# rg2/DeepFluoroLabeling-IPCAI2020

Hardware: AMD Instinct MI355X
Metric: train images/sec, paper U-Net (depth 6, wf 5, BN, strided-conv down, seg + 14-landmark heads), 1x192x192 (8x-downsampled 184x184 padded) (higher is better)
Workload: dtype bf16 (bf16 activations, activation gradients and GEMM weight copies in HBM; bf16 MFMA, fp32 accumulate, BatchNorm statistics, losses, weight gradients and master weights); 1 GPU; BASELINE configs[1]: 8x-downsampled, seg + 14-landmark heat-map dual head, batch 16 per GPU, Dice+NCC loss, SGD nesterov; global_batch=16, image=1x192x192, parallelism=dp1, math=bf16s, optimizer=dfl_amd.SGD(momentum 0.9, nesterov, wd 1e-4)

## Files before the change

### deepfluorolabeling-ipcai2020_amd/csrc/direct_small.hip

```cpp
#include "common.h"
#include "direct_small.h"

namespace dfl {

constexpr int DK = DIRECT_MAX_K;

struct Gather {
  int iy0, ix0, base;
};

struct PixCursor {
  int ox, oy, n;
  __device__ __forceinline__ void init(int m, int Hg, int Wg) {
    ox = m % Wg;
    const int t = m / Wg;
    oy = t % Hg;
    n = t / Hg;
  }
  __device__ __forceinline__ void advance(int step, int Hg, int Wg) {
    ox += step;
    while (ox >= Wg) {
      ox -= Wg;
      if (++oy == Hg) {
        oy = 0;
        ++n;
      }
    }
  }
  __device__ __forceinline__ Gather origin(int stride, int pad, int Hin, int Win) const {
    Gather g;
    g.iy0 = oy * stride - pad;
    g.ix0 = ox * stride - pad;
    g.base = n * Hin * Win;
    return g;
  }
};

template <bool BF>
__device__ __forceinline__ float4 ld4c(const float* base, int64_t elem) {
  if constexpr (BF) {
    const uint2 w = *reinterpret_cast<const uint2*>(reinterpret_cast<const unsigned short*>(base) + elem);
    return make_float4(__uint_as_float(w.x << 16), __uint_as_float(w.x & 0xffff0000u), __uint_as_float(w.y << 16),
                       __uint_as_float(w.y & 0xffff0000u));
  } else {
    return *reinterpret_cast<const float4*>(base + elem);
  }
}
template <bool BF>
__device__ __forceinline__ float4 st4c(float* base, int64_t elem, float4 v) {
  if constexpr (BF) {
    const bf16x2_t h0 = __builtin_convertvector((f32x2_t){v.x, v.y}, bf16x2_t), h1 = __builtin_convertvector((f32x2_t){v.z, v.w}, bf16x2_t);
    const uint2 w = make_uint2(__builtin_bit_cast(unsigned, h0), __builtin_bit_cast(unsigned, h1));
    *reinterpret_cast<uint2*>(reinterpret_cast<unsigned short*>(base) + elem) = w;
    return make_float4(__uint_as_float(w.x << 16), __uint_as_float(w.x & 0xffff0000u), __uint_as_float(w.y << 16),
                       __uint_as_float(w.y & 0xffff0000u));
  } else {
    *reinterpret_cast<float4*>(base + elem) = v;
    return v;
  }
}

template <int KH, int KW, int CIN, bool BF>
__global__ void __launch_bounds__(256) direct_conv_kernel(const dfl_conv_args a, int Mtot, int rows_per_block) {
  constexpr int K = KH * KW * CIN;
  static_assert(K <= DK, "window too large for the direct kernel");
  __shared__ float red[2][256][4];
  const int cq = a.Ntot / 4, PL = 256 / cq;
  const int q = threadIdx.x % cq, pl = threadIdx.x / cq;
  const int n0 = 4 * q;
  float w[K][4];
#pragma unroll
  for (int k = 0; k < K; ++k) {
#pragma unroll
    for (int j = 0; j < 4; ++j) w[k][j] = a.w[((int64_t)(k >> 2) * a.Ntot + n0 + j) * 4 + (k & 3)];
  }
  float bias[4] = {0.f, 0.f, 0.f, 0.f}, asc[4] = {1.f, 1.f, 1.f, 1.f}, ash[4] = {0.f, 0.f, 0.f, 0.f};
#pragma unroll
  for (int j = 0; j < 4; ++j) {
    if (a.bias != nullptr) bias[j] = a.bias[n0 + j];
    if (a.add_scale != nullptr) {
      asc[j] = a.add_scale[n0 + j];
      ash[j] = a.add_shift[n0 + j];
    }
  }
  if (a.add != nullptr && a.add_scale == nullptr && a.add_tot != nullptr) {
    __shared__ float atab[2][1024];
    for (int c = threadIdx.x; c < a.Ntot; c += 256)
      bn_live_affine(a.add_tot, a.add_gamma, a.add_beta, a.add_count, a.bn_eps, a.Ntot, c, &atab[0][c], &atab[1][c]);
    __syncthreads();
#pragma unroll
    for (int j = 0; j < 4; ++j) {
      asc[j] = atab[0][n0 + j];
      ash[j] = atab[1][n0 + j];
    }
  }
  float isc[CIN], ish[CIN];
#pragma unroll
  for (int c = 0; c < CIN; ++c) {
    isc[c] = (a.in_scale != nullptr) ? a.in_scale[c] : 1.f;
    ish[c] = (a.in_scale != nullptr) ? a.in_shift[c] : 0.f;
  }
  float s1[4] = {0.f, 0.f, 0.f, 0.f}, s2[4] = {0.f, 0.f, 0.f, 0.f};
  const int m_begin = blockIdx.x * rows_per_block;
  const int m_end = min(Mtot, m_begin + rows_per_block);
  PixCursor cur;
  cur.init(min(m_begin + pl, Mtot - 1), a.Hout, a.Wout);
  for (int m = m_begin + pl; m < m_end; m += PL, cur.advance(PL, a.Hout, a.Wout)) {
    const Gather g = cur.origin(a.stride, a.pad, a.Hin, a.Win);
    float acc[4] = {bias[0], bias[1], bias[2], bias[3]};
    float xv[K];
#pragma unroll
    for (int dy = 0; dy < KH; ++dy)
#pragma unroll
      for (int dx = 0; dx < KW; ++dx)
#pragma unroll
        for (int c = 0; c < CIN; ++c) {
          const int iy = g.iy0 + dy, ix = g.ix0 + dx;
          const bool ok = (unsigned)iy < (unsigned)a.Hin && (unsigned)ix < (unsigned)a.Win;
          const float x = a.x[ok ? ((int64_t)(g.base + iy * a.Win + ix) * a.ldx + c) : 0];
          xv[(dy * KW + dx) * CIN + c] = ok ? fmaf(x, isc[c], ish[c]) : 0.f;
        }
#pragma unroll
    for (int k = 0; k < K; ++k)
#pragma unroll
      for (int j = 0; j < 4; ++j) acc[j] = fmaf(xv[k], w[k][j], acc[j]);
    if (a.add != nullptr) {
      const float4 r = ld4c<BF>(a.add, (int64_t)m * a.ldadd + n0);
      acc[0] += fmaf(r.x, asc[0], ash[0]);
      acc[1] += fmaf(r.y, asc[1], ash[1]);
      acc[2] += fmaf(r.z, asc[2], ash[2]);
      acc[3] += fmaf(r.w, asc[3], ash[3]);
    }
    if (a.relu) {
#pragma unroll
      for (int j = 0; j < 4; ++j) acc[j] = fmaxf(acc[j], 0.f);
    }
    const int64_t yo = (int64_t)m * a.ldy + n0;
    if (a.accumulate) {
      const float4 o = ld4c<BF>(a.y, yo);
      acc[0] += o.x; acc[1] += o.y; acc[2] += o.z; acc[3] += o.w;
    }
    const float4 st = st4c<BF>(a.y, yo, make_float4(acc[0], acc[1], acc[2], acc[3]));
    acc[0] = st.x; acc[1] = st.y; acc[2] = st.z; acc[3] = st.w;
    if (a.stat_partials != nullptr) {
      float u[4] = {acc[0], acc[1], acc[2], acc[3]};
      if (a.stat_other != nullptr) {
        const float4 o = ld4c<BF>(a.stat_other, (int64_t)m * a.ldso + n0);
        u[0] = o.x; u[1] = o.y; u[2] = o.z; u[3] = o.w;
      }
#pragma unroll
      for (int j = 0; j < 4; ++j) {
        s1[j] += acc[j];
        s2[j] = fmaf(acc[j], u[j], s2[j]);
      }
    }
  }
  if (a.stat_partials == nullptr) return;
#pragma unroll
  for (int j = 0; j < 4; ++j) {
    red[0][threadIdx.x][j] = s1[j];
    red[1][threadIdx.x][j] = s2[j];
  }
  __syncthreads();
  if (pl == 0) {
#pragma unroll
    for (int j = 0; j < 4; ++j) {
      float t1 = 0.f, t2 = 0.f;
      for (int p = 0; p < PL; ++p) {
        t1 += red[0][p * cq + q][j];
        t2 += red[1][p * cq + q][j];
      }
      a.stat_partials[((int64_t)blockIdx.x * 2 + 0) * a.Ntot + n0 + j] = t1;
      a.stat_partials[((int64_t)blockIdx.x * 2 + 1) * a.Ntot + n0 + j] = t2;
    }
  }
}

template <bool BF>
__device__ __forceinline__ void ld8c(const float* base, int64_t elem, float* v) {
  if constexpr (BF) {
    const uint4 w = *reinterpret_cast<const uint4*>(reinterpret_cast<const unsigned short*>(base) + elem);
    v[0] = __uint_as_float(w.x << 16); v[1] = __uint_as_float(w.x & 0xffff0000u);
    v[2] = __uint_as_float(w.y << 16); v[3] = __uint_as_float(w.y & 0xffff0000u);
    v[4] = __uint_as_float(w.z << 16); v[5] = __uint_as_float(w.z & 0xffff0000u);
    v[6] = __uint_as_float(w.w << 16); v[7] = __uint_as_float(w.w & 0xffff0000u);
  } else {
    const float4 a = *reinterpret_cast<const float4*>(base + elem), b = *reinterpret_cast<const float4*>(base + elem + 4);
    v[0] = a.x; v[1] = a.y; v[2] = a.z; v[3] = a.w; v[4] = b.x; v[5] = b.y; v[6] = b.z; v[7] = b.w;
  }
}
template <bool BF>
__device__ __forceinline__ void st8c(float* base, int64_t elem, float* v) {
  if constexpr (BF) {
    uint4 w;
    w.x = __builtin_bit_cast(unsigned, __builtin_convertvector((f32x2_t){v[0], v[1]}, bf16x2_t));
    w.y = __builtin_bit_cast(unsigned, __builtin_convertvector((f32x2_t){v[2], v[3]}, bf16x2_t));
    w.z = __builtin_bit_cast(unsigned, __builtin_convertvector((f32x2_t){v[4], v[5]}, bf16x2_t));
    w.w = __builtin_bit_cast(unsigned, __builtin_convertvector((f32x2_t){v[6], v[7]}, bf16x2_t));
    *reinterpret_cast<uint4*>(reinterpret_cast<unsigned short*>(base) + elem) = w;
    v[0] = __uint_as_float(w.x << 16); v[1] = __uint_as_float(w.x & 0xffff0000u);
    v[2] = __uint_as_float(w.y << 16); v[3] = __uint_as_float(w.y & 0xffff0000u);
    v[4] = __uint_as_float(w.z << 16); v[5] = __uint_as_float(w.z & 0xffff0000u);
    v[6] = __uint_as_float(w.w << 16); v[7] = __uint_as_float(w.w & 0xffff0000u);
  } else {
    *reinterpret_cast<float4*>(base + elem) = make_float4(v[0], v[1], v[2], v[3]);
    *reinterpret_cast<float4*>(base + elem + 4) = make_float4(v[4], v[5], v[6], v[7]);
  }
}

#ifndef DFL_ROWS_CONV_RB
#define DFL_ROWS_CONV_RB 2
#endif
#ifndef DFL_ROWS_WGRAD_RB
#define DFL_ROWS_WGRAD_RB 4
#endif
#ifndef DFL_ROWS_CONV_BPB
#define DFL_ROWS_CONV_BPB 3
#endif
#ifndef DFL_ROWS_WGRAD_BPB
#define DFL_ROWS_WGRAD_BPB 1
#endif
constexpr int ROWS_CONV_BPB = DFL_ROWS_CONV_BPB, ROWS_WGRAD_BPB = DFL_ROWS_WGRAD_BPB;
constexpr int ROWS_CONV_RB = DFL_ROWS_CONV_RB, ROWS_WGRAD_RB = DFL_ROWS_WGRAD_RB;

template <bool BF>
__global__ void __launch_bounds__(256) direct_conv3_rows_kernel(const dfl_conv_args a) {
  __shared__ float red[2][256][8];
  const int cq = a.Ntot >> 3, PL = 256 / cq;
  const int q = threadIdx.x % cq, pl = threadIdx.x / cq;
  const int n0 = 8 * q;
  const int bands = (a.Hout + ROWS_CONV_RB - 1) / ROWS_CONV_RB;
  float w[9][8], bias[8], s1[8], s2[8];
#pragma unroll
  for (int j = 0; j < 8; ++j) {
#pragma unroll
    for (int k = 0; k < 9; ++k) w[k][j] = a.w[((int64_t)(k >> 2) * a.Ntot + n0 + j) * 4 + (k & 3)];
    bias[j] = a.bias != nullptr ? a.bias[n0 + j] : 0.f;
    s1[j] = 0.f;
    s2[j] = 0.f;
  }
  extern __shared__ float img_rows[];
  const int RW = a.Wout + 2;
  for (int bb = 0; bb < ROWS_CONV_BPB; ++bb) {
  const int band = (int)blockIdx.x * ROWS_CONV_BPB + bb;
  if (band >= a.N * bands) break;
  const int n = band / bands, y0 = (band - n * bands) * ROWS_CONV_RB;
  const float* img = a.x + (int64_t)n * a.Hin * a.Win * a.ldx;
  if (bb > 0) __syncthreads();
  for (int idx = threadIdx.x; idx < (ROWS_CONV_RB + 2) * RW; idx += 256) {
    const int r = idx / RW, c = idx - r * RW;
    const int iy = y0 - a.pad + r, ix = c - a.pad;
    const bool ok = (unsigned)iy < (unsigned)a.Hin && (unsigned)ix < (unsigned)a.Win;
    img_rows[idx] = ok ? img[(int64_t)(iy * a.Win + ix) * a.ldx] : 0.f;
  }
  __syncthreads();
#pragma unroll
  for (int ry = 0; ry < ROWS_CONV_RB; ++ry) {
    const int y = y0 + ry;
    if (y >= a.Hout) break;
    for (int x = pl; x < a.Wout; x += PL) {
      float xv[9];
#pragma unroll
      for (int dy = 0; dy < 3; ++dy)
#pragma unroll
        for (int dx = 0; dx < 3; ++dx) xv[dy * 3 + dx] = img_rows[(ry + dy) * RW + x + dx];
      float acc[8];
#pragma unroll
      for (int j = 0; j < 8; ++j) acc[j] = bias[j];
#pragma unroll
      for (int k = 0; k < 9; ++k)
#pragma unroll
        for (int j = 0; j < 8; ++j) acc[j] = fmaf(xv[k], w[k][j], acc[j]);
      if (a.relu) {
#pragma unroll
        for (int j = 0; j < 8; ++j) acc[j] = fmaxf(acc[j], 0.f);
      }
      st8c<BF>(a.y, ((int64_t)(n * a.Hout + y) * a.Wout + x) * a.ldy + n0, acc);
#pragma unroll
      for (int j = 0; j < 8; ++j) {
        s1[j] += acc[j];
        s2[j] = fmaf(acc[j], acc[j], s2[j]);
      }
    }
  }
  if (a.stat_partials != nullptr || a.stat_totals != nullptr) {
    __syncthreads();
#pragma unroll
    for (int j = 0; j < 8; ++j) {
      red[0][threadIdx.x][j] = s1[j];
      red[1][threadIdx.x][j] = s2[j];
      s1[j] = 0.f;
      s2[j] = 0.f;
    }
    __syncthreads();
    for (int idx = threadIdx.x; idx < 2 * a.Ntot; idx += 256) {
      const int which = idx / a.Ntot, c = idx - which * a.Ntot;
      const int qq = c >> 3, j = c & 7;
      float t = 0.f;
      for (int p = 0; p < PL; ++p) t += red[which][p * cq + qq][j];
      if (a.stat_totals != nullptr) bn_live_add(a.stat_totals, band, which, a.Ntot, c, t);
      else a.stat_partials[((int64_t)band * 2 + which) * a.Ntot + c] = t;
    }
  }
  }
}

static bool direct_conv_rows_ok(const dfl_conv_args* a) {
  return a->KH == 3 && a->KW == 3 && a->Cin == 1 && a->stride == 1 && a->add == nullptr && !a->accumulate && a->stat_other == nullptr &&
         a->in_scale == nullptr && a->Ntot % 8 == 0 && a->Ntot <= 64 && 256 % (a->Ntot / 8) == 0 && a->ldy % 8 == 0 && aligned16(a->y);
}

template <bool BF, bool DB = false>
__global__ void __launch_bounds__(256) direct_wgrad3_rows_kernel(const dfl_wgrad_args a) {
  __shared__ float red[4][8 * 72];
  const int cq = a.Cm >> 3, PL = 256 / cq;
  const int q = threadIdx.x % cq, pl = threadIdx.x / cq;
  const int bands = (a.Hout + ROWS_WGRAD_RB - 1) / ROWS_WGRAD_RB;
  float acc[9][8];
#pragma unroll
  for (int k = 0; k < 9; ++k)
#pragma unroll
    for (int j = 0; j < 8; ++j) acc[k][j] = 0.f;
  extern __shared__ float img_rows[];
  const int RW = a.Wout + 2;
  float cA[DB ? 8 : 1], cB[DB ? 8 : 1], cC[DB ? 8 : 1], bsum[DB ? 8 : 1];
  if constexpr (DB) {
    if (a.coef_tot != nullptr) {
      float* ctab = &red[0][0];
      if ((int)threadIdx.x < a.Cm)
        bn_live_coef(a.coef_tot, a.bn_gamma, a.bn_mean, a.bn_invstd, a.bn_count, a.Cm, (int)threadIdx.x, ctab + threadIdx.x, ctab + 64 + threadIdx.x,
                     ctab + 128 + threadIdx.x);
      __syncthreads();
#pragma unroll
      for (int j = 0; j < 8; ++j) {
        cA[j] = ctab[8 * q + j];
        cB[j] = ctab[64 + 8 * q + j];
        cC[j] = ctab[128 + 8 * q + j];
        bsum[j] = 0.f;
      }
      __syncthreads();
    } else {
#pragma unroll
      for (int j = 0; j < 8; ++j) {
        cA[j] = a.coef != nullptr ? a.coef[8 * q + j] : 1.f;
        cB[j] = a.coef != nullptr ? a.coef[a.Cm + 8 * q + j] : 0.f;
        cC[j] = a.coef != nullptr ? a.coef[2 * a.Cm + 8 * q + j] : 0.f;
        bsum[j] = 0.f;
      }
    }
  }
  for (int bb = 0; bb < ROWS_WGRAD_BPB; ++bb) {
  const int band = (int)blockIdx.x * ROWS_WGRAD_BPB + bb;
  if (band >= a.N * bands) break;
  const int n = band / bands, y0 = (band - n * bands) * ROWS_WGRAD_RB;
  const float* img = a.g + (int64_t)n * a.Hin * a.Win * a.ldg;
  if (bb > 0) __syncthreads();
  for (int idx = threadIdx.x; idx < (ROWS_WGRAD_RB + 2) * RW; idx += 256) {
    const int r = idx / RW, c = idx - r * RW;
    const int iy = y0 - a.pad + r, ix = c - a.pad;
    const bool ok = (unsigned)iy < (unsigned)a.Hin && (unsigned)ix < (unsigned)a.Win;
    img_rows[idx] = ok ? img[(int64_t)(iy * a.Win + ix) * a.ldg] : 0.f;
  }
  __syncthreads();
#pragma unroll
  for (int ry = 0; ry < ROWS_WGRAD_RB; ++ry) {
    const int y = y0 + ry;
    if (y >= a.Hout) break;
    for (int x = pl; x < a.Wout; x += PL) {
      float d[8], xv[9];
      ld8c<BF>(a.d, ((int64_t)(n * a.Hout + y) * a.Wout + x) * a.ldd + 8 * q, d);
      if constexpr (DB) {
        float r[8];
        ld8c<BF>(a.d2, ((int64_t)(n * a.Hout + y) * a.Wout + x) * a.ldd2 + 8 * q, r);
#pragma unroll
        for (int j = 0; j < 8; ++j) {
          const float v = r[j] > 0.f ? fmaf(cA[j], d[j], fmaf(cB[j], r[j], cC[j])) : 0.f;
          d[j] = (float)(__bf16)v;
          bsum[j] += d[j];
        }
      }
#pragma unroll
      for (int dy = 0; dy < 3; ++dy)
#pragma unroll
        for (int dx = 0; dx < 3; ++dx) xv[dy * 3 + dx] = img_rows[(ry + dy) * RW + x + dx];
#pragma unroll
      for (int k = 0; k < 9; ++k)
#pragma unroll
        for (int j = 0; j < 8; ++j) acc[k][j] = fmaf(xv[k], d[j], acc[k][j]);
    }
  }
  }
  const int lane = threadIdx.x & 63, wave = threadIdx.x >> 6;
#pragma unroll
  for (int k = 0; k < 9; ++k)
#pragma unroll
    for (int j = 0; j < 8; ++j) {
      float v = acc[k][j];
      for (int off = cq; off < 64; off <<= 1) v += __shfl_xor(v, off, 64);
      acc[k][j] = v;
    }
  if (lane < cq) {
#pragma unroll
    for (int k = 0; k < 9; ++k)
#pragma unroll
      for (int j = 0; j < 8; ++j) red[wave][(lane * 9 + k) * 8 + j] = acc[k][j];
  }
  __syncthreads();
  const bool sliced = a.splits > 1;
  float* out = sliced ? a.partial + (int64_t)blockIdx.x * a.Cm * 9 : a.dw;
  for (int idx = threadIdx.x; idx < cq * 72; idx += 256) {
    const float t = ((red[0][idx] + red[1][idx]) + red[2][idx]) + red[3][idx];
    const int qq = idx / 72, r = idx - qq * 72, k = r >> 3, j = r & 7;
    const int cm = 8 * qq + j;
    out[sliced ? (int64_t)k * a.Cm + cm : (int64_t)cm * 9 + k] = t;
  }
  if constexpr (DB) {
    if (a.bias_partial == nullptr) return;
#pragma unroll
    for (int j = 0; j < 8; ++j) {
      float v = bsum[j];
      for (int off = cq; off < 64; off <<= 1) v += __shfl_xor(v, off, 64);
      bsum[j] = v;
    }
    __syncthreads();
    if (lane < cq) {
#pragma unroll
      for (int j = 0; j < 8; ++j) red[wave][lane * 8 + j] = bsum[j];
    }
    __syncthreads();
    for (int idx = threadIdx.x; idx < a.Cm; idx += 256)
      a.bias_partial[(int64_t)blockIdx.x * a.Cm + idx] = ((red[0][idx] + red[1][idx]) + red[2][idx]) + red[3][idx];
  }
}

static bool direct_wgrad_rows_ok(const dfl_wgrad_args* a) {
  return a->KH == 3 && a->KW == 3 && a->Cg == 1 && a->stride == 1 && a->in_scale == nullptr && a->Cm % 8 == 0 && a->Cm <= 64 &&
         256 % (a->Cm / 8) == 0 && 64 % (a->Cm / 8) == 0 && a->ldd % 8 == 0 && aligned16(a->d) && !a->g_bf16;
}

static bool direct_window(int KH, int KW, int C) {
  if (KH != KW) return false;
  return (KH == 3 && C == 1) || (KH == 2 && C >= 1 && C <= 3) || (KH == 1 && C >= 1 && C <= 4);
}

bool direct_conv_rows_usable(const dfl_conv_args* a) { return direct_conv_rows_ok(a); }

bool direct_conv_ok(const dfl_conv_args* a) {
  if (!direct_window(a->KH, a->KW, a->Cin) || a->scatter2x2 || a->splits > 1) return false;
  if (a->Ntot % 4 != 0 || a->Ntot > 1024 || 256 % (a->Ntot / 4) != 0) return false;
  if (a->x_bf16) return false;
  if (a->ldy % 4 != 0 || !aligned16(a->y)) return false;
  if (a->add != nullptr && (a->ldadd % 4 != 0 || !aligned16(a->add))) return false;
  if (a->stat_other != nullptr && (a->ldso % 4 != 0 || !aligned16(a->stat_other))) return false;
  return true;
}

int direct_conv_blocks(const dfl_conv_args* a) {
  if (direct_conv_rows_ok(a)) return a->N * (int)ceil_div(a->Hout, ROWS_CONV_RB);
  const int64_t M = (int64_t)a->N * a->Hout * a->Wout;
  const int PL = 256 / (a->Ntot / 4);
  int64_t b = ceil_div(M, (int64_t)PL * 8);
  if (b > 2048) b = 2048;
  return (int)(b < 1 ? 1 : b);
}

int direct_conv_launch(const dfl_conv_args* a, hipStream_t s) {
  const int64_t M = (int64_t)a->N * a->Hout * a->Wout;
  const int blocks = direct_conv_blocks(a);
  if (direct_conv_rows_ok(a)) {
    const size_t lds = (size_t)(ROWS_CONV_RB + 2) * (a->Wout + 2) * sizeof(float);
    const unsigned wgs = (unsigned)ceil_div(blocks, ROWS_CONV_BPB);
    if (a->y_bf16) hipLaunchKernelGGL(direct_conv3_rows_kernel<true>, dim3(wgs), dim3(256), lds, s, *a);
    else hipLaunchKernelGGL(direct_conv3_rows_kernel<false>, dim3(wgs), dim3(256), lds, s, *a);
    return check_launch("dfl_conv2d");
  }
  const int rpb = (int)ceil_div(M, blocks);
#define DFL_DC(KH_, C_)                                                                                                  \
  {                                                                                                                      \
    if (a->y_bf16) hipLaunchKernelGGL((direct_conv_kernel<KH_, KH_, C_, true>), dim3((unsigned)blocks), dim3(256), 0, s, *a, (int)M, rpb);  \
    else hipLaunchKernelGGL((direct_conv_kernel<KH_, KH_, C_, false>), dim3((unsigned)blocks), dim3(256), 0, s, *a, (int)M, rpb);           \
  }
  switch (a->KH * 10 + a->Cin) {
    case 31: DFL_DC(3, 1); break;
    case 21: DFL_DC(2, 1); break;
    case 22: DFL_DC(2, 2); break;
    case 23: DFL_DC(2, 3); break;
    case 11: DFL_DC(1, 1); break;
    case 12: DFL_DC(1, 2); break;
    case 13: DFL_DC(1, 3); break;
    default: DFL_DC(1, 4); break;
  }
#undef DFL_DC
  return check_launch("dfl_conv2d");
}

template <int KH, int KW, int CG, bool BF>
__global__ void __launch_bounds__(256) direct_wgrad_kernel(const dfl_wgrad_args a, int Mtot, int rows_per_block) {
  constexpr int K = KH * KW * CG, T = KH * KW;
  static_assert(K <= DK, "window too large for the direct kernel");
  __shared__ float red[256][4];
  const int cq = a.Cm / 4, PL = 256 / cq;
  const int q = threadIdx.x % cq, pl = threadIdx.x / cq;
  const int Cg = CG;
  float isc[CG], ish[CG];
#pragma unroll
  for (int c = 0; c < CG; ++c) {
    isc[c] = (a.in_scale != nullptr) ? a.in_scale[c] : 1.f;
    ish[c] = (a.in_scale != nullptr) ? a.in_shift[c] : 0.f;
  }
  float acc[K][4];
#pragma unroll
  for (int k = 0; k < K; ++k)
#pragma unroll
    for (int j = 0; j < 4; ++j) acc[k][j] = 0.f;
  const int m_begin = blockIdx.x * rows_per_block;
  const int m_end = min(Mtot, m_begin + rows_per_block);
  PixCursor cur;
  cur.init(min(m_begin + pl, Mtot - 1), a.Hout, a.Wout);
  for (int m = m_begin + pl; m < m_end; m += PL, cur.advance(PL, a.Hout, a.Wout)) {
    const Gather g = cur.origin(a.stride, a.pad, a.Hin, a.Win);
    const float4 d = ld4c<BF>(a.d, (int64_t)m * a.ldd + 4 * q);
    float xv[K];
#pragma unroll
    for (int dy = 0; dy < KH; ++dy)
#pragma unroll
      for (int dx = 0; dx < KW; ++dx)
#pragma unroll
        for (int c = 0; c < CG; ++c) {
          const int iy = g.iy0 + dy, ix = g.ix0 + dx;
          const bool ok = (unsigned)iy < (unsigned)a.Hin && (unsigned)ix < (unsigned)a.Win;
          const float x = a.g[ok ? ((int64_t)(g.base + iy * a.Win + ix) * a.ldg + c) : 0];
          xv[(dy * KW + dx) * CG + c] = ok ? fmaf(x, isc[c], ish[c]) : 0.f;
        }
#pragma unroll
    for (int k = 0; k < K; ++k) {
      acc[k][0] = fmaf(xv[k], d.x, acc[k][0]);
      acc[k][1] = fmaf(xv[k], d.y, acc[k][1]);
      acc[k][2] = fmaf(xv[k], d.z, acc[k][2]);
      acc[k][3] = fmaf(xv[k], d.w, acc[k][3]);
    }
  }
  const bool sliced = a.splits > 1;
  float* out = sliced ? a.partial + (int64_t)blockIdx.x * a.Cm * a.Cg * T : a.dw;
#pragma unroll
  for (int k = 0; k < K; ++k) {
    __syncthreads();
#pragma unroll
    for (int j = 0; j < 4; ++j) red[threadIdx.x][j] = acc[k][j];
    __syncthreads();
    if (pl == 0) {
      const int t = k / Cg, cg = k - t * Cg;
#pragma unroll
      for (int j = 0; j < 4; ++j) {
        float s = 0.f;
        for (int p = 0; p < PL; ++p) s += red[p * cq + q][j];
        const int cm = 4 * q + j;
        out[sliced ? ((int64_t)t * a.Cm + cm) * Cg + cg : ((int64_t)cm * Cg + cg) * T + t] = s;
      }
    }
  }
}

bool direct_wgrad_ok(const dfl_wgrad_args* a) {
  if (!direct_window(a->KH, a->KW, a->Cg)) return false;
  if (a->Cm % 4 != 0 || a->Cm > 1024 || 256 % (a->Cm / 4) != 0) return false;
  if (a->ldd % 4 != 0 || !aligned16(a->d) || a->g_bf16) return false;
  return true;
}

int direct_wgrad_splits(const dfl_wgrad_args* a) {
  if (direct_wgrad_rows_ok(a)) return (int)ceil_div((int64_t)a->N * ceil_div(a->Hout, ROWS_WGRAD_RB), ROWS_WGRAD_BPB);
  const int64_t M = (int64_t)a->N * a->Hout * a->Wout;
  const int PL = 256 / (a->Cm / 4);
  int64_t b = ceil_div(M, (int64_t)PL * 16);
  if (b > 1024) b = 1024;
  return (int)(b < 1 ? 1 : b);
}

int direct_wgrad_launch(const dfl_wgrad_args* a, hipStream_t s) {
  if (direct_wgrad_rows_ok(a) && a->splits == direct_wgrad_splits(a)) {
    const size_t rows_lds = (size_t)(ROWS_WGRAD_RB + 2) * (a->Wout + 2) * sizeof(float);
    DFL_REQUIRE(a->coef_tot == nullptr || (a->d_mode == 1 && a->coef == nullptr && a->bn_gamma && a->bn_mean && a->bn_invstd && a->bn_count > 0),
                "dfl_conv2d_wgrad (1-channel 3x3): coef_tot replaces coef (d_mode 1) and needs bn_gamma, bn_mean, bn_invstd, bn_count");
    if (a->d_mode != 0) {
      DFL_REQUIRE(a->d_mode == 1 && a->d_bf16 && a->d2 != nullptr && a->ldd2 % 8 == 0 && aligned16(a->d2),
                  "dfl_conv2d_wgrad (1-channel 3x3): d_mode 1 needs bf16 d / d2 (16-byte aligned, ldd2 %% 8 == 0)");
      hipLaunchKernelGGL((direct_wgrad3_rows_kernel<true, true>), dim3((unsigned)a->splits), dim3(256), rows_lds, s, *a);
    } else if (a->d_bf16) {
      hipLaunchKernelGGL(direct_wgrad3_rows_kernel<true>, dim3((unsigned)a->splits), dim3(256), rows_lds, s, *a);
    } else {
      hipLaunchKernelGGL(direct_wgrad3_rows_kernel<false>, dim3((unsigned)a->splits), dim3(256), rows_lds, s, *a);
    }
    return check_launch("dfl_conv2d_wgrad");
  }
  DFL_REQUIRE(a->d_mode == 0, "dfl_conv2d_wgrad: d_mode is implemented by the bf16 patch kernels and the 1-channel 3x3 row form only");
  const int64_t M = (int64_t)a->N * a->Hout * a->Wout;
  const int rpb = (int)ceil_div(M, a->splits);
#define DFL_DW(KH_, C_)                                                                                                  \
  {                                                                                                                      \
    if (a->d_bf16) hipLaunchKernelGGL((direct_wgrad_kernel<KH_, KH_, C_, true>), dim3((unsigned)a->splits), dim3(256), 0, s, *a, (int)M, rpb);  \
    else hipLaunchKernelGGL((direct_wgrad_kernel<KH_, KH_, C_, false>), dim3((unsigned)a->splits), dim3(256), 0, s, *a, (int)M, rpb);           \
  }
  switch (a->KH * 10 + a->Cg) {
    case 31: DFL_DW(3, 1); break;
    case 21: DFL_DW(2, 1); break;
    case 22: DFL_DW(2, 2); break;
    case 23: DFL_DW(2, 3); break;
    case 11: DFL_DW(1, 1); break;
    case 12: DFL_DW(1, 2); break;
    case 13: DFL_DW(1, 3); break;
    default: DFL_DW(1, 4); break;
  }
#undef DFL_DW
  return check_launch("dfl_conv2d_wgrad");
}

}
```

### deepfluorolabeling-ipcai2020_amd/csrc/head_mfma.h

```cpp
#pragma once
#include "common.h"
#include "head_wgrad.h"

namespace dfl {

struct HFrag { bf16x8_t hi, lo; };

__device__ __forceinline__ HFrag hsplit8(const float* v) {
  HFrag f;
  float r[8];
#pragma unroll
  for (int e = 0; e < 8; ++e) {
    const __bf16 h = (__bf16)v[e];
    f.hi[e] = h;
    r[e] = v[e] - (float)h;
  }
#pragma unroll
  for (int e = 0; e < 8; ++e) f.lo[e] = (__bf16)r[e];
  return f;
}

__device__ __forceinline__ void hmm3(f32x16& acc, const HFrag& a, const HFrag& b) {
  acc = __builtin_amdgcn_mfma_f32_32x32x16_bf16(a.lo, b.hi, acc, 0, 0, 0);
  acc = __builtin_amdgcn_mfma_f32_32x32x16_bf16(a.hi, b.lo, acc, 0, 0, 0);
  acc = __builtin_amdgcn_mfma_f32_32x32x16_bf16(a.hi, b.hi, acc, 0, 0, 0);
}
__device__ __forceinline__ void hmm2(f32x16& acc, const HFrag& a, const bf16x8_t b) {
  acc = __builtin_amdgcn_mfma_f32_32x32x16_bf16(a.lo, b, acc, 0, 0, 0);
  acc = __builtin_amdgcn_mfma_f32_32x32x16_bf16(a.hi, b, acc, 0, 0, 0);
}

__device__ __forceinline__ void acc_to_b(const f32x16& acc, int s, float* v) {
#pragma unroll
  for (int j = 0; j < 4; ++j) {
    const auto r = __builtin_amdgcn_permlane32_swap(__float_as_uint(acc[8 * s + j]), __float_as_uint(acc[8 * s + 4 + j]), false, false);
    v[j] = __uint_as_float(r[0]);
    v[4 + j] = __uint_as_float(r[1]);
  }
}

struct HeadW {
  const float* w_seg; const float* w_l1; const float* w_l2;
  int NC, NM, L, K1;
  __device__ __forceinline__ float wseg(int c, int f) const { return c < NC ? w_seg[c * 32 + f] : 0.f; }
  __device__ __forceinline__ float w1x(int j, int f) const { return j < NM ? w_l1[j * K1 + f] : 0.f; }
  __device__ __forceinline__ float w1c(int j, int c) const { return (j < NM && c < NC) ? w_l1[j * K1 + 32 + c] : 0.f; }
  __device__ __forceinline__ float w2(int l, int j) const { return (l < L && j < NM) ? w_l2[l * NM + j] : 0.f; }
  __device__ __forceinline__ HFrag a_u(int m, int k0, bool lands) const {
    float v[8];
#pragma unroll
    for (int e = 0; e < 8; ++e) v[e] = m < 8 ? wseg(m, k0 + e) : (lands ? w1x(m - 8, k0 + e) : 0.f);
    if (lands && m >= 8 && m - 8 < NM) {
      for (int c = 0; c < NC; ++c) {
        const float wc = w_l1[(m - 8) * K1 + 32 + c];
        const float4 s0 = *reinterpret_cast<const float4*>(w_seg + c * 32 + k0), s1 = *reinterpret_cast<const float4*>(w_seg + c * 32 + k0 + 4);
        v[0] = fmaf(wc, s0.x, v[0]); v[1] = fmaf(wc, s0.y, v[1]); v[2] = fmaf(wc, s0.z, v[2]); v[3] = fmaf(wc, s0.w, v[3]);
        v[4] = fmaf(wc, s1.x, v[4]); v[5] = fmaf(wc, s1.y, v[5]); v[6] = fmaf(wc, s1.z, v[6]); v[7] = fmaf(wc, s1.w, v[7]);
      }
    }
    return hsplit8(v);
  }
  __device__ __forceinline__ HFrag a_h(int m, int k0) const {
    float v[8];
#pragma unroll
    for (int e = 0; e < 8; ++e) v[e] = (k0 + e >= 8) ? w2(m, k0 + e - 8) : 0.f;
    return hsplit8(v);
  }
  __device__ __forceinline__ HFrag a_dm(int m, int k0) const {
    float v[8];
#pragma unroll
    for (int e = 0; e < 8; ++e) v[e] = m >= 8 ? w2(k0 + e, m - 8) : 0.f;
    return hsplit8(v);
  }
  __device__ __forceinline__ HFrag a_dl(int m, int k0) const {
    float v[8];
#pragma unroll
    for (int e = 0; e < 8; ++e) v[e] = (m < 8 && k0 + e >= 8) ? w1c(k0 + e - 8, m) : 0.f;
    return hsplit8(v);
  }
  __device__ __forceinline__ HFrag a_dx(int m, int k0, bool lands) const {
    float v[8];
#pragma unroll
    for (int e = 0; e < 8; ++e) {
      const int r = k0 + e;
      v[e] = r < 8 ? wseg(r, m) : (lands ? w1x(r - 8, m) : 0.f);
    }
    return hsplit8(v);
  }
};

constexpr int HM_TILE = HEAD_WG_ROWS;

__device__ __forceinline__ bf16x8_t hload_x(const unsigned short* xb, int64_t m, int64_t M, int ldx, int s, int h) {
  uint4 w = make_uint4(0u, 0u, 0u, 0u);
  if (m < M) w = *reinterpret_cast<const uint4*>(xb + m * ldx + 16 * s + 8 * h);
  return __builtin_bit_cast(bf16x8_t, w);
}

template <bool LANDS>
__global__ void __launch_bounds__(256) head_mfma_fwd_kernel(const dfl_head_fwd_args a) {
  const int lane = threadIdx.x & 63, wave = threadIdx.x >> 6, l = lane & 31, h = lane >> 5;
  const HeadW W{a.w_seg, a.w_l1, a.w_l2, a.NC, a.NM, a.L, 32 + a.NC};
  HFrag au[2], ah[2];
#pragma unroll
  for (int s = 0; s < 2; ++s) {
    au[s] = W.a_u(l, 16 * s + 8 * h, LANDS);
    if (LANDS) ah[s] = W.a_h(l, 16 * s + 8 * h);
  }
  const unsigned short* xb = reinterpret_cast<const unsigned short*>(a.x);
  const int64_t HW = (int64_t)a.H * a.W, M = (int64_t)a.N * HW;
  const int64_t ntiles = (M + HM_TILE - 1) / HM_TILE;
  for (int64_t t = blockIdx.x; t < ntiles; t += gridDim.x) {
    const int64_t m = t * HM_TILE + wave * 32 + l;
    const bf16x8_t x0 = hload_x(xb, m, M, a.ldx, 0, h), x1 = hload_x(xb, m, M, a.ldx, 1, h);
    f32x16 u;
#pragma unroll
    for (int r = 0; r < 16; ++r) u[r] = 0.f;
    hmm2(u, au[0], x0);
    hmm2(u, au[1], x1);
    const int64_t n = m / HW, pp = m - n * HW;
    if (LANDS) {
      f32x16 ht;
#pragma unroll
      for (int r = 0; r < 16; ++r) ht[r] = 0.f;
#pragma unroll
      for (int s = 0; s < 2; ++s) {
        float v[8];
        acc_to_b(u, s, v);
        hmm3(ht, ah[s], hsplit8(v));
      }
      if (m < M) {
        float* hp = a.heat + n * a.L * HW + pp;
#pragma unroll
        for (int r = 0; r < 8; ++r) {
          const int row = mfma32_row(r, lane);
          if (row < a.L) hp[(int64_t)row * HW] = ht[r];
        }
      }
    }
    float lg[4];
#pragma unroll
    for (int j = 0; j < 4; ++j) lg[j] = u[j];
    if (a.softmax) {
      float mx = -INFINITY;
#pragma unroll
      for (int j = 0; j < 4; ++j)
        if (4 * h + j < a.NC) mx = fmaxf(mx, lg[j]);
      mx = fmaxf(mx, xor32(mx));
      float sum = 0.f;
#pragma unroll
      for (int j = 0; j < 4; ++j) {
        lg[j] = 4 * h + j < a.NC ? expf(lg[j] - mx) : 0.f;
        sum += lg[j];
      }
      sum += xor32(sum);
      const float inv = 1.0f / sum;
#pragma unroll
      for (int j = 0; j < 4; ++j) lg[j] *= inv;
    }
    if (m < M) {
      float* sp = a.seg + n * a.NC * HW + pp;
#pragma unroll
      for (int j = 0; j < 4; ++j)
        if (4 * h + j < a.NC) sp[(int64_t)(4 * h + j) * HW] = lg[j];
    }
  }
}

template <bool LANDS>
__global__ void __launch_bounds__(256) head_mfma_bwd_kernel(const dfl_head_bwd_args a) {
  extern __shared__ __attribute__((aligned(16))) unsigned char ab[];
  const int lane = threadIdx.x & 63, wave = threadIdx.x >> 6, l = lane & 31, h = lane >> 5;
  const bool lands = LANDS && a.dheat != nullptr;
  const HeadW W{a.w_seg, a.w_l1, a.w_l2, a.NC, a.NM, a.L, 32 + a.NC};
  HFrag au[2], adl[2], adx[2], adm;
#pragma unroll
  for (int s = 0; s < 2; ++s) {
    au[s] = W.a_u(l, 16 * s + 8 * h, LANDS);
    adx[s] = W.a_dx(l, 16 * s + 8 * h, LANDS);
    if (LANDS) adl[s] = W.a_dl(l, 16 * s + 8 * h);
  }
  if (LANDS) adm = W.a_dm(l, 8 * h);
  const HeadWgLane wg;
  f32x16 wacc;
#pragma unroll
  for (int r = 0; r < 16; ++r) wacc[r] = 0.f;
  unsigned char* myrow = ab + (size_t)(wave * 32 + l) * HEAD_WG_PITCH;
  *reinterpret_cast<uint4*>(myrow + HEAD_WG_ZERO + 16 * h) = make_uint4(0u, 0u, 0u, 0u);
  const unsigned short* xb = reinterpret_cast<const unsigned short*>(a.x);
  unsigned short* dxb = reinterpret_cast<unsigned short*>(a.dx);
  const unsigned short* sob = reinterpret_cast<const unsigned short*>(a.stat_other);
  float st1[16], st2[16];
#pragma unroll
  for (int q = 0; q < 16; ++q) st1[q] = st2[q] = 0.f;
  const int64_t HW = (int64_t)a.H * a.W, M = (int64_t)a.N * HW;
  const int64_t ntiles = (M + HM_TILE - 1) / HM_TILE;
  for (int64_t t = blockIdx.x; t < ntiles; t += gridDim.x) {
    const int64_t m = t * HM_TILE + wave * 32 + l;
    const bool live = m < M;
    const int64_t n = m / HW, pp = m - n * HW;
    const bf16x8_t x0 = hload_x(xb, m, M, a.ldx, 0, h), x1 = hload_x(xb, m, M, a.ldx, 1, h);
    float dh[8], g[4], sv[4];
#pragma unroll
    for (int e = 0; e < 8; ++e) dh[e] = (lands && live && 8 * h + e < a.L) ? a.dheat[(n * a.L + 8 * h + e) * HW + pp] : 0.f;
#pragma unroll
    for (int j = 0; j < 4; ++j) {
      const bool ok = live && 4 * h + j < a.NC;
      g[j] = ok ? a.dseg[(n * a.NC + 4 * h + j) * HW + pp] : 0.f;
      sv[j] = ok ? a.seg[(n * a.NC + 4 * h + j) * HW + pp] : 0.f;
    }
    f32x16 u, v;
#pragma unroll
    for (int r = 0; r < 16; ++r) u[r] = v[r] = 0.f;
    hmm2(u, au[0], x0);
    hmm2(u, au[1], x1);
    const HFrag dhf = hsplit8(dh);
    if (LANDS) {
      hmm3(v, adm, dhf);
#pragma unroll
      for (int s = 0; s < 2; ++s) {
        float t8[8];
        acc_to_b(v, s, t8);
        hmm3(v, adl[s], hsplit8(t8));
      }
    }
    {
      float dot = 0.f;
#pragma unroll
      for (int j = 0; j < 4; ++j) dot = fmaf(g[j], sv[j], dot);
      dot += xor32(dot);
#pragma unroll
      for (int j = 0; j < 4; ++j) v[j] += a.softmax ? sv[j] * (g[j] - dot) : g[j];
    }
    f32x16 dx;
#pragma unroll
    for (int r = 0; r < 16; ++r) dx[r] = 0.f;
    HFrag vf[2];
    bf16x8_t uf[2];
#pragma unroll
    for (int s = 0; s < 2; ++s) {
      float t8[8];
      acc_to_b(v, s, t8);
      vf[s] = hsplit8(t8);
      hmm3(dx, adx[s], vf[s]);
      acc_to_b(u, s, t8);
#pragma unroll
      for (int e = 0; e < 8; ++e) uf[s][e] = (__bf16)t8[e];
    }
    __syncthreads();
#pragma unroll
    for (int s = 0; s < 2; ++s) {
      *reinterpret_cast<bf16x8_t*>(myrow + HEAD_WG_V + 32 * s + 16 * h) = vf[s].hi;
      *reinterpret_cast<bf16x8_t*>(myrow + HEAD_WG_U + 32 * s + 16 * h) = uf[s];
    }
    *reinterpret_cast<bf16x8_t*>(myrow + HEAD_WG_DHEAT + 16 * h) = dhf.hi;
    *reinterpret_cast<bf16x8_t*>(myrow + HEAD_WG_X + 16 * h) = x0;
    *reinterpret_cast<bf16x8_t*>(myrow + HEAD_WG_X + 32 + 16 * h) = x1;
    if (live) {
#pragma unroll
      for (int s = 0; s < 2; ++s) {
        float t8[8];
        acc_to_b(dx, s, t8);
        const u32x4 w = pack8(t8);
        *reinterpret_cast<u32x4*>(dxb + m * a.lddx + 16 * s + 8 * h) = w;
        if (a.stat_totals != nullptr) {
          const u32x4 rr = *reinterpret_cast<const u32x4*>(sob + m * a.ldso + 16 * s + 8 * h);
#pragma unroll
          for (int e2 = 0; e2 < 4; ++e2) {
            st1[8 * s + 2 * e2] += bf_lo(w[e2]);
            st1[8 * s + 2 * e2 + 1] += bf_hi(w[e2]);
            st2[8 * s + 2 * e2] = fmaf(bf_lo(w[e2]), bf_lo(rr[e2]), st2[8 * s + 2 * e2]);
            st2[8 * s + 2 * e2 + 1] = fmaf(bf_hi(w[e2]), bf_hi(rr[e2]), st2[8 * s + 2 * e2 + 1]);
          }
        }
      }
    }
    __syncthreads();
    wg.product(ab, wacc);
  }
  if (a.stat_totals != nullptr) {
    __syncthreads();
    float* sred = reinterpret_cast<float*>(ab);
#pragma unroll
    for (int q = 0; q < 32; ++q) {
      float v = q < 16 ? st1[q] : st2[q - 16];
#pragma unroll
      for (int off = 1; off < 32; off <<= 1) v += __shfl_xor(v, off, 64);
      if (l == 0) sred[(wave * 2 + h) * 32 + q] = v;
    }
    __syncthreads();
    if (threadIdx.x < 64) {
      const int which = threadIdx.x >> 5, s_ = (threadIdx.x >> 4) & 1, hh = (threadIdx.x >> 3) & 1, e = threadIdx.x & 7;
      const int q = which * 16 + s_ * 8 + e;
      const float t = ((sred[(0 * 2 + hh) * 32 + q] + sred[(1 * 2 + hh) * 32 + q]) + sred[(2 * 2 + hh) * 32 + q]) + sred[(3 * 2 + hh) * 32 + q];
      bn_live_add(a.stat_totals, (int)blockIdx.x, which, 32, 16 * s_ + 8 * hh + e, t);
    }
  }
  wg.store(a.wg_partial, wacc);
}

}
```

Before: 4878 images/sec.

## Prefetch next tile in head MFMA kernels and stage conv weights in LDS

The head forward and backward MFMA kernels now software-pipeline their grid-stride loops, loading the next tile's inputs (x, dheat, dseg, seg, BN partner rows) before computing the current tile, which hides global-load latency. The backward kernel also gets a waves-per-EU attribute to make room for the extra registers. The direct 3x3 rows conv kernel loads weights and bias cooperatively into shared memory before filling per-thread registers, restructures the image-row staging loop to drop the per-element divide, and lowers the default bands per block from 3 to 2. The cost is higher register pressure and possible occupancy loss from the prefetch buffers, plus an extra LDS table and barrier in the conv kernel.

```diff
diff --git a/deepfluorolabeling-ipcai2020_amd/csrc/direct_small.hip b/deepfluorolabeling-ipcai2020_amd/csrc/direct_small.hip
--- a/deepfluorolabeling-ipcai2020_amd/csrc/direct_small.hip
+++ b/deepfluorolabeling-ipcai2020_amd/csrc/direct_small.hip
@@ -215,7 +215,7 @@
 #define DFL_ROWS_WGRAD_RB 4
 #endif
 #ifndef DFL_ROWS_CONV_BPB
-#define DFL_ROWS_CONV_BPB 3
+#define DFL_ROWS_CONV_BPB 2
 #endif
 #ifndef DFL_ROWS_WGRAD_BPB
 #define DFL_ROWS_WGRAD_BPB 1
@@ -232,12 +232,17 @@
   const int bands = (a.Hout + ROWS_CONV_RB - 1) / ROWS_CONV_RB;
   float w[9][8], bias[8], s1[8], s2[8];
 #pragma unroll
+  for (int j = 0; j < 8; ++j) s1[j] = s2[j] = 0.f;
+  __shared__ __attribute__((aligned(16))) float wtab[3 * 64 * 4 + 64];
+  for (int idx = threadIdx.x; idx < 12 * a.Ntot; idx += 256)
+    if (idx < 8 * a.Ntot || (idx & 3) == 0) wtab[idx] = a.w[idx];
+  for (int idx = threadIdx.x; idx < a.Ntot; idx += 256) wtab[3 * 64 * 4 + idx] = a.bias != nullptr ? a.bias[idx] : 0.f;
+  __syncthreads();
+#pragma unroll
   for (int j = 0; j < 8; ++j) {
 #pragma unroll
-    for (int k = 0; k < 9; ++k) w[k][j] = a.w[((int64_t)(k >> 2) * a.Ntot + n0 + j) * 4 + (k & 3)];
-    bias[j] = a.bias != nullptr ? a.bias[n0 + j] : 0.f;
-    s1[j] = 0.f;
-    s2[j] = 0.f;
+    for (int k = 0; k < 9; ++k) w[k][j] = wtab[((k >> 2) * a.Ntot + n0 + j) * 4 + (k & 3)];
+    bias[j] = wtab[3 * 64 * 4 + n0 + j];
   }
   extern __shared__ float img_rows[];
   const int RW = a.Wout + 2;
@@ -247,11 +252,15 @@
   const int n = band / bands, y0 = (band - n * bands) * ROWS_CONV_RB;
   const float* img = a.x + (int64_t)n * a.Hin * a.Win * a.ldx;
   if (bb > 0) __syncthreads();
-  for (int idx = threadIdx.x; idx < (ROWS_CONV_RB + 2) * RW; idx += 256) {
-    const int r = idx / RW, c = idx - r * RW;
-    const int iy = y0 - a.pad + r, ix = c - a.pad;
-    const bool ok = (unsigned)iy < (unsigned)a.Hin && (unsigned)ix < (unsigned)a.Win;
-    img_rows[idx] = ok ? img[(int64_t)(iy * a.Win + ix) * a.ldx] : 0.f;
+#pragma unroll
+  for (int r = 0; r < ROWS_CONV_RB + 2; ++r) {
+    const int iy = y0 - a.pad + r;
+    const bool row_ok = (unsigned)iy < (unsigned)a.Hin;
+    for (int c = threadIdx.x; c < RW; c += 256) {
+      const int ix = c - a.pad;
+      const bool ok = row_ok && (unsigned)ix < (unsigned)a.Win;
+      img_rows[r * RW + c] = ok ? img[(int64_t)(iy * a.Win + ix) * a.ldx] : 0.f;
+    }
   }
   __syncthreads();
 #pragma unroll
diff --git a/deepfluorolabeling-ipcai2020_amd/csrc/head_mfma.h b/deepfluorolabeling-ipcai2020_amd/csrc/head_mfma.h
--- a/deepfluorolabeling-ipcai2020_amd/csrc/head_mfma.h
+++ b/deepfluorolabeling-ipcai2020_amd/csrc/head_mfma.h
@@ -110,14 +110,18 @@
   const unsigned short* xb = reinterpret_cast<const unsigned short*>(a.x);
   const int64_t HW = (int64_t)a.H * a.W, M = (int64_t)a.N * HW;
   const int64_t ntiles = (M + HM_TILE - 1) / HM_TILE;
-  for (int64_t t = blockIdx.x; t < ntiles; t += gridDim.x) {
-    const int64_t m = t * HM_TILE + wave * 32 + l;
-    const bf16x8_t x0 = hload_x(xb, m, M, a.ldx, 0, h), x1 = hload_x(xb, m, M, a.ldx, 1, h);
+  const int64_t mstep = (int64_t)gridDim.x * HM_TILE;
+  int64_t m = (int64_t)blockIdx.x * HM_TILE + wave * 32 + l;
+  bf16x8_t x0 = hload_x(xb, m, M, a.ldx, 0, h), x1 = hload_x(xb, m, M, a.ldx, 1, h);
+  for (int64_t t = blockIdx.x; t < ntiles; t += gridDim.x, m += mstep) {
+    const bf16x8_t nx0 = hload_x(xb, m + mstep, M, a.ldx, 0, h), nx1 = hload_x(xb, m + mstep, M, a.ldx, 1, h);
     f32x16 u;
 #pragma unroll
     for (int r = 0; r < 16; ++r) u[r] = 0.f;
     hmm2(u, au[0], x0);
     hmm2(u, au[1], x1);
+    x0 = nx0;
+    x1 = nx1;
     const int64_t n = m / HW, pp = m - n * HW;
     if (LANDS) {
       f32x16 ht;
@@ -167,11 +171,46 @@
   }
 }
 
+struct HeadBwdIn {
+  bf16x8_t x0, x1;
+  float dh[8], g[4], sv[4];
+  u32x4 rr[2];
+};
+
 template <bool LANDS>
-__global__ void __launch_bounds__(256) head_mfma_bwd_kernel(const dfl_head_bwd_args a) {
+__device__ __forceinline__ HeadBwdIn hbwd_load(const dfl_head_bwd_args& a, int64_t m, int64_t M, int64_t HW, int h) {
+  const unsigned short* xb = reinterpret_cast<const unsigned short*>(a.x);
+  const unsigned short* sob = reinterpret_cast<const unsigned short*>(a.stat_other);
+  const bool lands = LANDS && a.dheat != nullptr;
+  const bool live = m < M;
+  const int64_t n = m / HW, pp = m - n * HW;
+  HeadBwdIn in;
+  in.x0 = hload_x(xb, m, M, a.ldx, 0, h);
+  in.x1 = hload_x(xb, m, M, a.ldx, 1, h);
+#pragma unroll
+  for (int e = 0; e < 8; ++e) in.dh[e] = (lands && live && 8 * h + e < a.L) ? a.dheat[(n * a.L + 8 * h + e) * HW + pp] : 0.f;
+#pragma unroll
+  for (int j = 0; j < 4; ++j) {
+    const bool ok = live && 4 * h + j < a.NC;
+    in.g[j] = ok ? a.dseg[(n * a.NC + 4 * h + j) * HW + pp] : 0.f;
+    in.sv[j] = ok ? a.seg[(n * a.NC + 4 * h + j) * HW + pp] : 0.f;
+  }
+#pragma unroll
+  for (int s = 0; s < 2; ++s) {
+    in.rr[s] = (u32x4)(0u);
+    if (live && a.stat_totals != nullptr) in.rr[s] = *reinterpret_cast<const u32x4*>(sob + m * a.ldso + 16 * s + 8 * h);
+  }
+  return in;
+}
+
+#ifndef DFL_HEAD_MFMA_BWD_WAVES
+#define DFL_HEAD_MFMA_BWD_WAVES 2
+#endif
+
+template <bool LANDS>
+__global__ void __launch_bounds__(256) __attribute__((amdgpu_waves_per_eu(DFL_HEAD_MFMA_BWD_WAVES))) head_mfma_bwd_kernel(const dfl_head_bwd_args a) {
   extern __shared__ __attribute__((aligned(16))) unsigned char ab[];
   const int lane = threadIdx.x & 63, wave = threadIdx.x >> 6, l = lane & 31, h = lane >> 5;
-  const bool lands = LANDS && a.dheat != nullptr;
   const HeadW W{a.w_seg, a.w_l1, a.w_l2, a.NC, a.NM, a.L, 32 + a.NC};
   HFrag au[2], adl[2], adx[2], adm;
 #pragma unroll
@@ -187,28 +226,22 @@
   for (int r = 0; r < 16; ++r) wacc[r] = 0.f;
   unsigned char* myrow = ab + (size_t)(wave * 32 + l) * HEAD_WG_PITCH;
   *reinterpret_cast<uint4*>(myrow + HEAD_WG_ZERO + 16 * h) = make_uint4(0u, 0u, 0u, 0u);
-  const unsigned short* xb = reinterpret_cast<const unsigned short*>(a.x);
   unsigned short* dxb = reinterpret_cast<unsigned short*>(a.dx);
-  const unsigned short* sob = reinterpret_cast<const unsigned short*>(a.stat_other);
   float st1[16], st2[16];
 #pragma unroll
   for (int q = 0; q < 16; ++q) st1[q] = st2[q] = 0.f;
   const int64_t HW = (int64_t)a.H * a.W, M = (int64_t)a.N * HW;
   const int64_t ntiles = (M + HM_TILE - 1) / HM_TILE;
-  for (int64_t t = blockIdx.x; t < ntiles; t += gridDim.x) {
-    const int64_t m = t * HM_TILE + wave * 32 + l;
+  const int64_t mstep = (int64_t)gridDim.x * HM_TILE;
+  int64_t m = (int64_t)blockIdx.x * HM_TILE + wave * 32 + l;
+  HeadBwdIn cur = hbwd_load<LANDS>(a, m, M, HW, h);
+  for (int64_t t = blockIdx.x; t < ntiles; t += gridDim.x, m += mstep) {
     const bool live = m < M;
-    const int64_t n = m / HW, pp = m - n * HW;
-    const bf16x8_t x0 = hload_x(xb, m, M, a.ldx, 0, h), x1 = hload_x(xb, m, M, a.ldx, 1, h);
-    float dh[8], g[4], sv[4];
-#pragma unroll
-    for (int e = 0; e < 8; ++e) dh[e] = (lands && live && 8 * h + e < a.L) ? a.dheat[(n * a.L + 8 * h + e) * HW + pp] : 0.f;
-#pragma unroll
-    for (int j = 0; j < 4; ++j) {
-      const bool ok = live && 4 * h + j < a.NC;
-      g[j] = ok ? a.dseg[(n * a.NC + 4 * h + j) * HW + pp] : 0.f;
-      sv[j] = ok ? a.seg[(n * a.NC + 4 * h + j) * HW + pp] : 0.f;
-    }
+    const HeadBwdIn nxt = hbwd_load<LANDS>(a, m + mstep, M, HW, h);
+    const bf16x8_t x0 = cur.x0, x1 = cur.x1;
+    const float* dh = cur.dh;
+    const float* g = cur.g;
+    const float* sv = cur.sv;
     f32x16 u, v;
 #pragma unroll
     for (int r = 0; r < 16; ++r) u[r] = v[r] = 0.f;
@@ -264,7 +297,7 @@
         const u32x4 w = pack8(t8);
         *reinterpret_cast<u32x4*>(dxb + m * a.lddx + 16 * s + 8 * h) = w;
         if (a.stat_totals != nullptr) {
-          const u32x4 rr = *reinterpret_cast<const u32x4*>(sob + m * a.ldso + 16 * s + 8 * h);
+          const u32x4 rr = cur.rr[s];
 #pragma unroll
           for (int e2 = 0; e2 < 4; ++e2) {
             st1[8 * s + 2 * e2] += bf_lo(w[e2]);
@@ -277,6 +310,7 @@
     }
     __syncthreads();
     wg.product(ab, wacc);
+    cur = nxt;
   }
   if (a.stat_totals != nullptr) {
     __syncthreads();
```

Result: no change. 4893 images/sec (median of 5 runs) (+0.3%).
